# HKU-BAL/Clair

Hardware: AMD Instinct MI355X
Metric: candidate sites/sec (whole node) (higher is better)
Workload: dtype f32 (matmuls as 2-way fp16 split on MFMA with fp32 accumulate; gates/activations fp32); 1 GPU; ONT 122HD34 weights-shape model (random init), synthetic ont-profile pileup tensors, batch=1024, 4 batches in flight per GPU, inputs resident in HBM; batch=1024, streams=4, candidates_total=38912, device_warm_steps=251, collective=none (1 rank), transport=none

## Files before the change

clair_amd/csrc/engine.hip:

```cpp
#include "../../include/clair_amd.h"

#include <hip/hip_runtime.h>
#include <ctype.h>

#include <algorithm>
#include <atomic>
#include <cmath>
#include <cstdarg>
#include <cstdio>
#include <cstdlib>
#include <condition_variable>
#include <cstring>
#include <deque>
#include <list>
#include <memory>
#include <mutex>
#include <string>
#include <thread>
#include <vector>

#include "common.hip.h"
#include "dense.hip.h"
#include "decode.hip.h"
#include "evaluate.hip.h"
// ... 1178 lines not shown
    if (check_source_range(t, "clair_sites_add_rows", first, n)) return 1;
    if (fused_possible(e)) return fail(e, "clair_sites_add_rows is not available on a handle with the fused layer-2 launch: unset CLAIR_AMD_LSTM2_FUSED");
    HIP_TRY(e, hipSetDevice(e->device));
    Slot &s = e->slots[0];
    if (s.pending_n) return fail(e, "slot 0 still has a pending submit; call clair_wait first");
    if (ensure_slot_decode(e, s) || ensure_slot_sites(e, s)) return 1;
    Lane &l = *e->lanes[s.lane];
    std::lock_guard<std::mutex> g(l.order);
    HIP_TRY(e, hipMemcpyAsync(s.d_out.p, probs, (size_t)n * OUT_FLOATS * sizeof(float), hipMemcpyHostToDevice, l.stream));
    if (x) HIP_TRY(e, hipMemcpyAsync(s.d_x.p, x, (size_t)n * SITE_X * sizeof(float), hipMemcpyHostToDevice, l.stream));
    if (centre) HIP_TRY(e, hipMemcpyAsync(s.d_centre.p, centre, (size_t)n * 2, hipMemcpyHostToDevice, l.stream));
    else HIP_TRY(e, hipMemsetAsync(s.d_centre.p, 0, (size_t)n * 2, l.stream));
    if (seq) HIP_TRY(e, hipMemcpyAsync(s.d_seq.p, seq, (size_t)n * SITE_SEQ, hipMemcpyHostToDevice, l.stream));
    else HIP_TRY(e, hipMemsetAsync(s.d_seq.p, 0, (size_t)n * SITE_SEQ, l.stream));
    if (enqueue_sites_adopt(e, l, s, t, first, n, x != nullptr) || enqueue_sites_accumulate(e, l, s, t, first, n)) return 1;
    HIP_TRY(e, hipStreamSynchronize(l.stream));
    return read_overflow(t, "clair_sites_add_rows");
}

int clair_sites_finish(clair_sites_t *t, int min_count, int order, int64_t *n_out) {
    if (check_sites(t, "clair_sites_finish", false)) return 1;
    clair_engine *e = t->e;
    if (order != CLAIR_SITES_ORDER_CHAIN && order != CLAIR_SITES_ORDER_POSITION) return fail(e, "clair_sites_finish: order %d is neither chain (0) nor position (1)", order);
    HIP_TRY(e, hipSetDevice(e->device));
    if (quiesce(e)) return 1;
    if (read_overflow(t, "clair_sites_finish")) return 1;
    Lane &l = *e->lanes[0];
    std::lock_guard<std::mutex> g(l.order);
    const int64_t ns = t->n_sites;
    uint32_t kept = 0;
    if (ns > 0) {
        const int64_t *idx_row = order == CLAIR_SITES_ORDER_POSITION ? t->idx_row[t->cur].as<int64_t>() : nullptr;
        const unsigned blocks = (unsigned)((ns + 255) / 256);
        HIP_TRY(e, t->keep.ensure((size_t)ns * sizeof(uint32_t)));
        HIP_TRY(e, t->out_before.ensure((size_t)(ns + 1) * sizeof(uint32_t)));
        hipLaunchKernelGGL(sites_keep_kernel, dim3(blocks), dim3(256), 0, l.stream, t->count.as<int>(), idx_row, ns, std::max(min_count, 1), t->keep.as<uint32_t>());
        hipLaunchKernelGGL(sites_scan_kernel, dim3(1), dim3(256), 0, l.stream, t->keep.as<uint32_t>(), ns, t->out_before.as<uint32_t>());
        HIP_TRY(e, hipGetLastError());
        HIP_TRY(e, hipMemcpyAsync(&kept, t->out_before.as<uint32_t>() + ns, sizeof kept, hipMemcpyDeviceToHost, l.stream));
        HIP_TRY(e, hipStreamSynchronize(l.stream));
        if (kept) {
            HIP_TRY(e, t->out_row.ensure((size_t)kept * sizeof(int64_t)));
            HIP_TRY(e, t->out_key.ensure((size_t)kept * sizeof(int64_t)));
            HIP_TRY(e, t->out_count.ensure((size_t)kept * sizeof(int)));
            HIP_TRY(e, t->out_seq.ensure((size_t)kept * SITE_SEQ));
            HIP_TRY(e, t->avg.ensure((size_t)kept * OUT_FLOATS * sizeof(float)));
            hipLaunchKernelGGL(sites_compact_kernel, dim3(blocks), dim3(256), 0, l.stream, t->rows(), idx_row, ns, t->keep.as<uint32_t>(), t->out_before.as<uint32_t>(),
                               t->out_row.as<int64_t>(), t->out_key.as<int64_t>(), t->out_count.as<int>(), t->out_seq.as<unsigned char>());
            const int64_t n_values = (int64_t)kept * OUT_FLOATS;
            hipLaunchKernelGGL(sites_average_kernel, dim3((unsigned)((n_values + 255) / 256)), dim3(256), 0, l.stream, t->rows(), t->out_row.as<int64_t>(), n_values,
                               t->avg.as<float>());
            HIP_TRY(e, hipGetLastError());
            HIP_TRY(e, hipStreamSynchronize(l.stream));
        }
    }
    t->finished = true;
    t->n_out = kept;
    if (n_out) *n_out = kept;
    return 0;
}

int clair_sites_info(clair_sites_t *t, int64_t first, int64_t n, int64_t *positions, int32_t *counts, uint8_t *seq) {
    if (check_sites(t, "clair_sites_info", false) || check_output_range(t, "clair_sites_info", first, n)) return 1;
    clair_engine *e = t->e;
    HIP_TRY(e, hipSetDevice(e->device));
    if (n == 0) return 0;
    if (positions) HIP_TRY(e, hipMemcpy(positions, t->out_key.as<int64_t>() + first, (size_t)n * sizeof(int64_t), hipMemcpyDeviceToHost));
    if (counts) HIP_TRY(e, hipMemcpy(counts, t->out_count.as<int>() + first, (size_t)n * sizeof(int), hipMemcpyDeviceToHost));
    if (seq) HIP_TRY(e, hipMemcpy(seq, t->out_seq.as<unsigned char>() + (size_t)first * SITE_SEQ, (size_t)n * SITE_SEQ, hipMemcpyDeviceToHost));
    return 0;
}

int clair_sites_rows(clair_sites_t *t, int64_t first, int64_t n, float *out) {
    if (check_sites(t, "clair_sites_rows", false) || check_output_range(t, "clair_sites_rows", first, n)) return 1;
    clair_engine *e = t->e;
    if (n > 0 && !out) return fail(e, "clair_sites_rows: out is NULL");
    HIP_TRY(e, hipSetDevice(e->device));
    if (n > 0) HIP_TRY(e, hipMemcpy(out, t->avg.as<float>() + (size_t)first * OUT_FLOATS, (size_t)n * OUT_FLOATS * sizeof(float), hipMemcpyDeviceToHost));
    return 0;
}

int clair_sites_windows(clair_sites_t *t, int64_t first, int64_t n, float *x) {
    if (check_sites(t, "clair_sites_windows", false) || check_output_range(t, "clair_sites_windows", first, n)) return 1;
    clair_engine *e = t->e;
    if (n > INT32_MAX || (n > 0 && !x)) return fail(e, "clair_sites_windows: bad arguments");
    if (n == 0) return 0;
    HIP_TRY(e, hipSetDevice(e->device));
    if (quiesce(e)) return 1;
    Lane &l = *e->lanes[0];
    std::lock_guard<std::mutex> g(l.order);
    if (t->gathered.bytes < (size_t)n * SITE_X * sizeof(float)) HIP_TRY(e, t->gathered.ensure((size_t)n * SITE_X * sizeof(float)));
    hipLaunchKernelGGL(sites_gather_kernel, dim3((unsigned)((n + 3) / 4)), dim3(256), 0, l.stream, t->rows(), t->out_row.as<int64_t>(), t->avg.as<float>(), first, (int)n,
                       t->gathered.as<float>(), (unsigned char *)nullptr, (float *)nullptr);
    HIP_TRY(e, hipGetLastError());
    HIP_TRY(e, hipMemcpyAsync(x, t->gathered.p, (size_t)n * SITE_X * sizeof(float), hipMemcpyDeviceToHost, l.stream));
    HIP_TRY(e, hipStreamSynchronize(l.stream));
    return 0;
}

int clair_submit_site_calls(clair_engine_t *e, int slot, clair_sites_t *t, int64_t first, int n, clair_call_t *calls, float *gt21, float *genotype, float *l1, float *l2) {
    if (check_sites(t, "clair_submit_site_calls", false)) return 1;
    if (e != t->e) return fail(e, "clair_submit_site_calls: the site table belongs to another engine");
    if (check_slot(e, slot, false) || check_n(e, n)) return 1;
    if ((gt21 || genotype || l1 || l2) && !(gt21 && genotype && l1 && l2)) return fail(e, "the four probability arrays come together or not at all");
    if (!gt21 && !calls) return fail(e, "nothing asked for: neither call records nor probabilities");
    if (check_output_range(t, "clair_submit_site_calls", first, n)) return 1;
    if (fused_possible(e)) return fail(e, "clair_submit_site_calls runs on the two-launch layer-2 path only: unset CLAIR_AMD_LSTM2_FUSED");
    HIP_TRY(e, hipSetDevice(e->device));
    Slot &s = e->slots[slot];
    if (s.pending_n) return fail(e, "slot %d still has a pending submit; call clair_wait first", slot);
    if (ensure_slot_decode(e, s)) return 1;
    Lane &l = *e->lanes[s.lane];
    s.o_gt21 = gt21; s.o_gt = genotype; s.o_l1 = l1; s.o_l2 = l2;
    s.o_calls = calls;
    s.refetch = false;
    s.staged = 0;
    const bool same_out = s.cout == l.stream;
    {
        std::lock_guard<std::mutex> g(l.order);
        hipLaunchKernelGGL(sites_gather_kernel, dim3((n + 3) / 4), dim3(256), 0, l.stream, t->rows(), t->out_row.as<int64_t>(), t->avg.as<float>(), first, n, s.d_x.as<float>(),
                           s.d_centre.as<unsigned char>(), s.d_out.as<float>());
        HIP_TRY(e, hipGetLastError());
        if (calls && enqueue_decode(e, l, s, n)) return 1;
        if (same_out) { if (enqueue_results(e, l, s, n, calls != nullptr, gt21 != nullptr)) return 1; }
        else HIP_TRY(e, hipEventRecord(s.ev_done, l.stream));
    }
    if (!same_out) {
        HIP_TRY(e, hipStreamWaitEvent(s.cout, s.ev_done, 0));
        if (enqueue_results(e, l, s, n, calls != nullptr, gt21 != nullptr)) return 1;
    }
    s.pending_n = n;
    return 0;
}

int clair_predict(clair_engine_t *e, const float *x, int n, float *gt21, float *genotype, float *l1, float *l2) {
    if (clair_submit(e, 0, x, n, gt21, genotype, l1, l2)) return 1;
    return clair_wait(e, 0);
}

int clair_dataset_alloc(clair_engine_t *e, int64_t N, void **x_dev, void **out_dev) {
    if (!e) return fail(nullptr, "engine is NULL");
    if (N < 1 || !x_dev || !out_dev) return fail(e, "bad arguments to clair_dataset_alloc");
    HIP_TRY(e, hipSetDevice(e->device));
    const size_t rows = (size_t)N + e->max_pad;
    HIP_TRY(e, hipMalloc(x_dev, rows * CLAIR_INPUT_FLOATS * sizeof(float)));
    HIP_TRY(e, hipMemset(*x_dev, 0, rows * CLAIR_INPUT_FLOATS * sizeof(float)));
    HIP_TRY(e, hipMalloc(out_dev, rows * OUT_FLOATS * sizeof(float)));
    HIP_TRY(e, hipMemset(*out_dev, 0, rows * OUT_FLOATS * sizeof(float)));
    return 0;
}

int clair_dataset_free(clair_engine_t *e, void *x_dev, void *out_dev) {
    if (!e) return fail(nullptr, "engine is NULL");
    HIP_TRY(e, hipSetDevice(e->device));
    HIP_TRY(e, hipDeviceSynchronize());
    HIP_TRY(e, hipFree(x_dev));
    HIP_TRY(e, hipFree(out_dev));
    return 0;
}

int clair_dataset_upload(clair_engine_t *e, void *x_dev, int64_t first, const float *x_host, int64_t n) {
    if (!e) return fail(nullptr, "engine is NULL");
    HIP_TRY(e, hipSetDevice(e->device));
    HIP_TRY(e, hipMemcpy((float *)x_dev + (size_t)first * CLAIR_INPUT_FLOATS, x_host, (size_t)n * CLAIR_INPUT_FLOATS * sizeof(float), hipMemcpyHostToDevice));
    return 0;
}

int clair_dataset_download(clair_engine_t *e, const void *out_dev, int64_t first, float *out_host, int64_t n) {
    if (!e) return fail(nullptr, "engine is NULL");
    HIP_TRY(e, hipSetDevice(e->device));
    HIP_TRY(e, hipMemcpy(out_host, (const float *)out_dev + (size_t)first * OUT_FLOATS, (size_t)n * OUT_FLOATS * sizeof(float), hipMemcpyDeviceToHost));
    return 0;
}

int clair_run_resident(clair_engine_t *e, int slot, const void *x_dev, void *out_dev, int64_t first, int n) {
    if (check_slot(e, slot) || check_n(e, n)) return 1;
    HIP_TRY(e, hipSetDevice(e->device));
    Lane &l = *e->lanes[e->slots[slot].lane];
    std::lock_guard<std::mutex> g(l.order);
    return enqueue_forward(e, l, *e->models[0], (const float *)x_dev + (size_t)first * CLAIR_INPUT_FLOATS, (float *)out_dev + (size_t)first * OUT_FLOATS, n, -1);
}

int clair_sync(clair_engine_t *e) {
    if (!e) return fail(nullptr, "engine is NULL");
    HIP_TRY(e, hipSetDevice(e->device));
    if (quiesce(e)) return 1;
    return check_fused_placement(e);
}

int clair_timing_enable(clair_engine_t *e, int on) {
    if (!e) return fail(nullptr, "engine is NULL");
    HIP_TRY(e, hipSetDevice(e->device));
    if (drain_timers(e)) return 1;
    e->timing_mask = on == 0 ? 0u : (on == 1 ? ~0u : (unsigned)on);
    return 0;
}

int clair_kernel_times(clair_engine_t *e, double *ms_sum, int64_t *launches) {
    if (!e) return fail(nullptr, "engine is NULL");
    HIP_TRY(e, hipSetDevice(e->device));
    if (drain_timers(e)) return 1;
    for (int k = 0; k < CLAIR_K_COUNT; ++k) {
        if (ms_sum) ms_sum[k] = e->ms_sum[k];
        if (launches) launches[k] = e->launches[k];
    }
    return 0;
}

int clair_timing_reset(clair_engine_t *e) {
    if (!e) return fail(nullptr, "engine is NULL");
    HIP_TRY(e, hipSetDevice(e->device));
    if (drain_timers(e)) return 1;
    for (int k = 0; k < CLAIR_K_COUNT; ++k) { e->ms_sum[k] = 0; e->launches[k] = 0; }
    return 0;
}

int clair_kernel_workgroups(clair_engine_t *e, int n, int *workgroups) {
    if (!e) return fail(nullptr, "engine is NULL");
    if (!workgroups) return fail(e, "workgroups is NULL");
    if (n < 1 || n > e->max_batch) return fail(e, "n %d out of range [1,%d]", n, e->max_batch);
    const int n_pad = (n + 31) & ~31, ntiles = n_pad / 32;
    const int x_tiles = (T_POS * n_pad + GS_ROWS - 1) / GS_ROWS;
    for (int k = 0; k < CLAIR_K_COUNT; ++k) workgroups[k] = 0;
    workgroups[CLAIR_K_LSTM1] = ntiles * 2;
    workgroups[CLAIR_K_LSTM2] = use_lstm2_pair(e, ntiles) ? ((ntiles + 1) / 2) * 2 : ntiles * 2;
    workgroups[CLAIR_K_PROJ2] = 32 * std::min(e->proj2_groups, (x_tiles + 7) / 8);
    if (use_lstm2_fused(e, ntiles)) {
        workgroups[CLAIR_K_LSTM2] = 32 * e->fused_groups + 32 * ((ntiles / 2 + 7) / 8);
        workgroups[CLAIR_K_PROJ2] = 0;
    }
    workgroups[CLAIR_K_L4] = l34_grid((n_pad + L34_CAND - 1) / L34_CAND);
    workgroups[CLAIR_K_TAIL] = n_pad / TAIL_TILE;
    workgroups[CLAIR_K_DECODE] = (n + 3) / 4;
    return 0;
}

int clair_pinned_alloc(clair_engine_t *e, int64_t bytes, void **ptr) {
    if (!e) return fail(nullptr, "engine is NULL");
    if (!ptr || bytes < 1) return fail(e, "bad arguments to clair_pinned_alloc");
    HIP_TRY(e, hipSetDevice(e->device));
    std::list<PinnedBuffer> one(1);
    HIP_TRY(e, one.front().ensure((size_t)bytes));
    *ptr = one.front().p;
    std::lock_guard<std::mutex> g(e->pinned_mu);
    e->pinned.splice(e->pinned.end(), one);
    return 0;
}

int clair_pinned_free(clair_engine_t *e, void *ptr) {
    if (!e) return fail(nullptr, "engine is NULL");
    bool known = false;
    {
        std::lock_guard<std::mutex> g(e->pinned_mu);
        for (const auto &b : e->pinned) known |= b.p == ptr;
    }
    if (!known) return fail(e, "clair_pinned_free: not a buffer of clair_pinned_alloc");
    HIP_TRY(e, hipSetDevice(e->device));
    if (quiesce(e)) return 1;
    std::lock_guard<std::mutex> g(e->pinned_mu);
    e->pinned.remove_if([ptr](const PinnedBuffer &b) { return b.p == ptr; });
    return 0;
}

int clair_engine_counter(clair_engine_t *e, int which, int64_t *value) {
    if (!e) return fail(nullptr, "engine is NULL");
    if (!value) return fail(e, "value is NULL");
    switch (which) {
        case 0: *value = e->fused_launches; return 0;
        case 1: *value = e->fused_recoveries; return 0;
        default: return fail(e, "clair_engine_counter: unknown counter %d", which);
    }
}

int clair_debug_read(clair_engine_t *e, int slot, int which, float *host, int64_t count) {
    if (check_slot(e, slot)) return 1;
    HIP_TRY(e, hipSetDevice(e->device));
    if (quiesce(e)) return 1;
    Lane &l = *e->lanes[e->slots[slot].lane];
    const float *src = nullptr;
    int64_t avail = 0;
    const int64_t np = l.last_n_pad;
    if (which == 1) {
        avail = (int64_t)T_POS * np * 256;
        if (count > avail) return fail(e, "clair_debug_read: asked %lld floats, tap 1 holds %lld", (long long)count, (long long)avail);
        std::vector<unsigned short> planes((size_t)2 * avail);
        HIP_TRY(e, hipMemcpy(planes.data(), l.a1.p, planes.size() * sizeof(unsigned short), hipMemcpyDeviceToHost));
        for (int64_t i = 0; i < count; ++i) host[i] = f16_value(planes[i]) + f16_value(planes[avail + i]);
        return 0;
    }
    if (which == 2) {
        avail = (int64_t)T_POS * np * 256;
        if (count > avail) return fail(e, "clair_debug_read: asked %lld floats, tap 2 holds %lld", (long long)count, (long long)avail);
        std::vector<float> raw((size_t)avail);
        HIP_TRY(e, hipMemcpy(raw.data(), l.a2.p, raw.size() * sizeof(float), hipMemcpyDeviceToHost));
        for (int64_t i = 0; i < count; ++i) {
            const int64_t t = i / (np * 256), n = (i / 256) % np, c = i % 256;
            host[i] = raw[(size_t)((((c / 8) * T_POS + t) * np + n) * 8 + c % 8)];
        }
        return 0;
    }
    switch (which) {
        case 4: if (!e->tap_l3) return fail(e, "clair_debug_read: tap 4 needs CLAIR_AMD_TAP_L3=1 at engine creation");
                src = l.zx.as<float>(); avail = np * L3_OUT; break;
        case 5: if (!e->l34_stamps) return fail(e, "clair_debug_read: tap 5 needs CLAIR_AMD_L34_STAMPS=1 at engine creation");
                src = l.zx.as<float>(); avail = ((np + L34_CAND - 1) / L34_CAND) * L4_SPLITS * 8 * 16 * 2; break;
        case 3: {
            avail = (int64_t)L4_SPLITS * np * L4_UNITS;
            if (count > avail) return fail(e, "clair_debug_read: asked %lld floats, tap 3 holds %lld", (long long)count, (long long)avail);
            const int64_t nblk = (np + L34_CAND - 1) / L34_CAND;
            std::vector<float> raw((size_t)L4_SPLITS * nblk * L34_CAND * L4_UNITS);
            HIP_TRY(e, hipMemcpy(raw.data(), l.l4part.p, raw.size() * sizeof(float), hipMemcpyDeviceToHost));
            const float inv = std::ldexp(1.0f, -e->models[0]->w4_shift) / L34_ACT_SCALE;
            for (int64_t i = 0; i < count; ++i) {
                const int64_t cg = i / (np * L4_UNITS), n = (i / L4_UNITS) % np, col = i % L4_UNITS;
                const int64_t blk = n / 64, row = n % 64, mb = row / 32, a = (row % 32) / 8, hq = (row % 8) / 4, r = row % 4;
                const int64_t nh = col / 96, nb = (col % 96) / 32, l32 = col % 32;
                host[i] = raw[(size_t)((((((cg * nblk + blk) * 2 + nh) * 6 + mb * 3 + nb) * 4 + a) * 64 + hq * 32 + l32) * 4 + r)] * inv;
            }
            return 0;
        }
        default: return fail(e, "clair_debug_read: unknown tap %d", which);
    }
    if (count > avail) return fail(e, "clair_debug_read: asked %lld floats, tap %d holds %lld", (long long)count, which, (long long)avail);
    HIP_TRY(e, hipMemcpy(host, src, (size_t)count * sizeof(float), hipMemcpyDeviceToHost));
    return 0;
}

}
```

clair_amd/csrc/gemm_split.hip.h:

```cpp
#pragma once
#include "common.hip.h"
#include "lstm32.hip.h"
#include <type_traits>

namespace clair {

typedef unsigned short f16bits_t;

struct GemmSplitArgs {
    const f16bits_t *X3;
    const f16bits_t *W3;
    const float *bias;
    float *C;
    int n_pad;
    int ntiles;
    int m_rows;
    int groups;
};

constexpr int GS_ROWS = 64;
constexpr int GS_PLANE = GS_ROWS * 32;
constexpr int GS_PHASE = 2 * 2 * GS_PLANE;

__device__ __forceinline__ int split_lds_off(int row, int chunk) { return row * 32 + ((chunk ^ ((row >> 3) & 3)) << 3); }

constexpr int GS_RING = 4;

template <bool FUSED>
__device__ __forceinline__ void gemm_split_body(const GemmSplitArgs &p, const int block, const FuseArgs &fz) {
    __shared__ __attribute__((aligned(16))) f16bits_t Xs[GS_RING][GS_PHASE];

    const int tid = threadIdx.x;
    const int lane = tid & 63;
    const int wave = __builtin_amdgcn_readfirstlane(tid >> 6);
    const int l32 = lane & 31, lh = lane >> 5;
    const int xcd = block & 7, local = block >> 3;
    const int gtile = local & 3, group = local >> 2;
    const int x_tiles = (p.m_rows + GS_ROWS - 1) / GS_ROWS;
    const int x_step = 8 * p.groups;
    const int x_first = xcd + 8 * group;
    const int npairs = p.ntiles >> 1;
    const int nq = FUSED ? (xcd < npairs ? (npairs - xcd + 7) >> 3 : 0) : 0;
    const int n_items = T_POS * nq;
    if (FUSED ? group >= n_items : x_first >= x_tiles) return;
    const int n_my = FUSED ? (n_items - group + p.groups - 1) / p.groups : (x_tiles - x_first + x_step - 1) / x_step;
    const int slice = gtile * 4 + wave;
    auto xt_of = [&](int it) -> int {
        if (!FUSED) return x_first + it * x_step;
        const int i = group + it * p.groups, s_ = i / nq, k = i - s_ * nq;
        return ((gtile >> 1) ? T_POS - 1 - s_ : s_) * npairs + xcd + 8 * k;
    };

    f16x8 Wr[2][16][2];
    {
        const f16x8 *wp = (const f16x8 *)p.W3 + ((size_t)slice * (2 * 16 * 2 * 64)) + lane;
#pragma unroll
        for (int mi = 0; mi < 2; ++mi)
#pragma unroll
            for (int kk = 0; kk < 16; ++kk)
#pragma unroll
                for (int pl = 0; pl < 2; ++pl) Wr[mi][kk][pl] = wp[((mi * 16 + kk) * 2 + pl) * 64];
#pragma unroll
        for (int mi = 0; mi < 2; ++mi)
#pragma unroll
            for (int kk = 0; kk < 16; ++kk)
#pragma unroll
                for (int pl = 0; pl < 2; ++pl) asm volatile("" : "+a"(Wr[mi][kk][pl]));
    }
    f32x4 bq[2][4];
#pragma unroll
    for (int mi = 0; mi < 2; ++mi)
#pragma unroll
        for (int a = 0; a < 4; ++a) bq[mi][a] = *(const f32x4 *)(p.bias + slice * 64 + mi * 32 + 8 * a + 4 * lh);
#pragma unroll
    for (int mi = 0; mi < 2; ++mi)
#pragma unroll
        for (int a = 0; a < 4; ++a) asm volatile("" : "+v"(bq[mi][a]));
    CLAIR_VMWAIT(0);

    const int my_slab = wave >> 1, my_plane = wave & 1;
    unsigned lane_off[4];
#pragma unroll
    for (int j = 0; j < 4; ++j) {
        const int row = 16 * j + (lane >> 2), c = (lane & 3) ^ ((row >> 3) & 3);
        lane_off[j] = (unsigned)(row * 512 + c * 16);
    }
    const f16bits_t *my_base = p.X3 + (size_t)my_plane * p.m_rows * 256 + my_slab * 32;
    const unsigned lds0 = __builtin_amdgcn_readfirstlane((unsigned)(size_t)(lptr_t)&Xs[0][0]) + (unsigned)(wave * GS_PLANE * 2);
    const int n_phases = n_my * 4;
    auto phase_base = [&](int P) -> const f16bits_t * {
        const int q = P < n_phases ? P : n_phases - 1;
        return my_base + ((size_t)xt_of(q >> 2) * GS_ROWS * 256) + (q & 3) * 64;
    };
    auto dma = [&](int P, int j) { glds16_s(lane_off[j], phase_base(P), lds0 + (unsigned)((P & (GS_RING - 1)) * GS_PHASE * 2 + j * 1024)); };
    auto fread = [&](f16x8 (&xf)[2][2][2], int slot, int sl) {
#pragma unroll
        for (int kk = 0; kk < 2; ++kk)
#pragma unroll
            for (int pl = 0; pl < 2; ++pl)
#pragma unroll
                for (int ni = 0; ni < 2; ++ni)
                    xf[kk][pl][ni] = *(const f16x8 *)&Xs[slot][(sl * 2 + pl) * GS_PLANE + split_lds_off(ni * 32 + l32, 2 * kk + lh)];
    };

    auto fread1 = [&](f16x8 (&xf)[2][2][2], int slot, int sl, int i) {
        const int kk = i >> 2, pl = (i >> 1) & 1, ni = i & 1;
        xf[kk][pl][ni] = *(const f16x8 *)&Xs[slot][(sl * 2 + pl) * GS_PLANE + split_lds_off(ni * 32 + l32, 2 * kk + lh)];
    };

    f16x8 xa[2][2][2], xb[2][2][2];
#pragma unroll
    for (int P = 0; P < 3; ++P)
#pragma unroll
        for (int j = 0; j < 4; ++j) dma(P, j);
    CLAIR_VMWAIT(8);
    __syncthreads();
    fread(xa, 0, 0);

    f32x16 accs[2][2][2];
    f32x16 bias16[2];
#pragma unroll
    for (int mi = 0; mi < 2; ++mi)
#pragma unroll
        for (int a = 0; a < 4; ++a) {
            bias16[mi][4 * a] = bq[mi][a][0]; bias16[mi][4 * a + 1] = bq[mi][a][1];
            bias16[mi][4 * a + 2] = bq[mi][a][2]; bias16[mi][4 * a + 3] = bq[mi][a][3];
        }
    asm volatile("" : "+v"(bias16[0]), "+v"(bias16[1]));
    size_t gate_off[2];
#pragma unroll
    for (int mi = 0; mi < 2; ++mi) {
        const int gblk = slice * 2 + mi;
        gate_off[mi] = ((size_t)(gblk >> 4) * p.ntiles * T_POS * 16 + (gblk & 15)) * 1024;
    }
    auto tile_off = [&](int xt, int ni) -> size_t {
        const int xblk = xt * 2 + ni;
        const int t = xblk / p.ntiles, tile = xblk - t * p.ntiles;
        return ((size_t)tile * T_POS + t) * 16 * 1024;
    };
    auto store_piece = [&](const f32x16 (&acc)[2][2], const size_t (&toff)[2], int j) {
        const int ni = j >> 3, mi = (j >> 2) & 1, a = j & 3;
        f32x4 *dst = (f32x4 *)(p.C + gate_off[mi] + toff[ni] + a * 256) + lane;
        __builtin_nontemporal_store((f32x4){acc[mi][ni][4 * a], acc[mi][ni][4 * a + 1], acc[mi][ni][4 * a + 2], acc[mi][ni][4 * a + 3]}, dst);
    };
    auto publish = [&](int xt) {
        if (!FUSED) return;
        const int t = xt / npairs, q = xt - t * npairs;
        unsigned *fw = fz.flags + (((size_t)((gtile >> 1) * p.ntiles + 2 * q) * T_POS + t) * 8) + (gtile & 1) * 4 + wave;
        if (lane == 0) {
            __hip_atomic_store(fw, fz.ticket, __ATOMIC_RELAXED, __HIP_MEMORY_SCOPE_AGENT);
            __hip_atomic_store(fw + T_POS * 8, fz.ticket, __ATOMIC_RELAXED, __HIP_MEMORY_SCOPE_AGENT);
        }
    };
    auto run_tile = [&](auto set_c, auto first_c, int it) {
        constexpr int SET = decltype(set_c)::value;
        constexpr bool FIRST_TILE = decltype(first_c)::value;
        f32x16 (&acc)[2][2] = accs[SET];
        const int xt_prev = xt_of(FIRST_TILE ? 0 : it - 1);
        const size_t toff[2] = {tile_off(xt_prev, 0), tile_off(xt_prev, 1)};
#pragma unroll
        for (int ph = 0; ph < 4; ++ph) {
            const int P = it * 4 + ph;
#pragma unroll
            for (int m = 0; m < 24; ++m) {
                const int kk = m / 12, term = (m % 12) / 4, mi = (m >> 1) & 1, ni = m & 1;
                if (ph == 0 && m < 4) mfma32_av_first(acc[mi][ni], Wr[mi][0][1], xa[0][0][ni], bias16[mi]);
                else mfma32_av(acc[mi][ni], Wr[mi][ph * 4 + kk][term == 0 ? 1 : 0], xa[kk][term == 1 ? 1 : 0][ni]);
                __builtin_amdgcn_sched_barrier(0);
                CLAIR_DBG_FENCE();
                if (m < 8) fread1(xb, ph, 1, m);
                __builtin_amdgcn_sched_barrier(0);
            }
            CLAIR_VMWAIT(4);
            __syncthreads();
            if (FUSED && ph == 3 && !FIRST_TILE) publish(xt_prev);
#pragma unroll
            for (int m = 0; m < 24; ++m) {
                const int kk = m / 12, term = (m % 12) / 4, mi = (m >> 1) & 1, ni = m & 1;
                mfma32_av(acc[mi][ni], Wr[mi][ph * 4 + 2 + kk][term == 0 ? 1 : 0], xb[kk][term == 1 ? 1 : 0][ni]);
                __builtin_amdgcn_sched_barrier(0);
                CLAIR_DBG_FENCE();
                if (m < 8) fread1(xa, (ph + 1) & 3, 0, m);
                if (!FIRST_TILE && ph < 2 && m >= 1 && m <= 8) store_piece(accs[SET ^ 1], toff, ph * 8 + m - 1);
                if (m >= 10 && m < 18 && (m & 1) == 0) dma(P + 3, (m - 10) >> 1);
                __builtin_amdgcn_sched_barrier(0);
            }
        }
    };
    run_tile(std::integral_constant<int, 0>(), std::true_type(), 0);
    for (int it = 1; it < n_my; it += 2) {
        run_tile(std::integral_constant<int, 1>(), std::false_type(), it);
        if (it + 1 < n_my) run_tile(std::integral_constant<int, 0>(), std::false_type(), it + 1);
    }
    {
        const int last = n_my - 1, xt = xt_of(last);
        const size_t toff[2] = {tile_off(xt, 0), tile_off(xt, 1)};
        asm volatile("s_nop 11" : "+v"(accs[0][0][0]), "+v"(accs[0][0][1]), "+v"(accs[0][1][0]), "+v"(accs[0][1][1]),
                                  "+v"(accs[1][0][0]), "+v"(accs[1][0][1]), "+v"(accs[1][1][0]), "+v"(accs[1][1][1]));
#pragma unroll
        for (int j = 0; j < 16; ++j) {
            if ((xt * 2 + (j >> 3)) * 32 >= p.m_rows) continue;
            if (last & 1) store_piece(accs[1], toff, j); else store_piece(accs[0], toff, j);
        }
    }
    CLAIR_VMWAIT(0);
    if (FUSED) publish(xt_of(n_my - 1));
}

__global__ __launch_bounds__(256) __attribute__((amdgpu_waves_per_eu(1, 1))) void gemm_split_kernel(GemmSplitArgs p) {
    gemm_split_body<false>(p, blockIdx.x, FuseArgs{nullptr, 0u, nullptr, nullptr});
}

}
```

clair_amd/csrc/weight_images.h:

```cpp
#pragma once
#include "../../include/clair_amd.h"

#include <algorithm>
#include <cmath>
#include <cstddef>
#include <cstring>
#include <vector>

namespace clair {

struct LayerSizes {
    int t_pos, f_in, hid, l3_units, l4_units, l5_units;
    int l34_groups, l34_ks, l34_ch;
    int l32_x_shift;
};

constexpr int HEAD_SIZE[4] = {CLAIR_GT21, CLAIR_GENOTYPE, CLAIR_INDEL_LEN, CLAIR_INDEL_LEN};

constexpr int64_t TENSOR_COUNT[CLAIR_T_COUNT] = {
    160 * 512, 512, 160 * 512, 512, 384 * 512, 512, 384 * 512, 512, 256 * 33 * 30, 256 * 30,
    7680 * 192, 192, 4 * 192 * 96, 4 * 96, 96 * HEAD_SIZE[0], HEAD_SIZE[0], 96 * HEAD_SIZE[1], HEAD_SIZE[1],
    96 * HEAD_SIZE[2], HEAD_SIZE[2], 96 * HEAD_SIZE[3], HEAD_SIZE[3]};

inline unsigned short f16_bits(_Float16 h) { unsigned short u; memcpy(&u, &h, 2); return u; }
inline float f16_value(unsigned short u) { _Float16 h; memcpy(&h, &u, 2); return (float)h; }
inline void split2_host(float x, unsigned short &hi, unsigned short &lo) {
    const _Float16 h = (_Float16)x;
    const _Float16 l = (_Float16)(x - (float)h);
    hi = f16_bits(h);
    lo = f16_bits(l);
}

inline float gate_scale(int col512) {
    const float L2E = 1.44269504088896340736f;
    return ((col512 >> 7) == 1) ? 2.0f * L2E : -L2E;
}

inline int gate_col(int w, int b, int rho) {
    const int a = rho >> 3, hq = (rho >> 2) & 1, c = rho & 3;
    return c * 128 + 32 * w + 8 * b + 4 * hq + a;
}

inline int image_shift(float vmax) {
    if (!(vmax > 0.0f) || !std::isfinite(vmax)) return 0;
    int ex = 0;
    (void)std::frexp(vmax, &ex);
    return std::max(-20, std::min(40, 14 - ex));
}
inline float max_abs(const float *v, size_t n, float vmax = 0.0f) {
    for (size_t i = 0; i < n; ++i) vmax = std::max(vmax, std::fabs(v[i]));
    return vmax;
}

struct SplitImage {
    std::vector<unsigned short> data;
    explicit SplitImage(size_t frags) : data(frags * 2 * 64 * 8, 0) {}
    void put(size_t frag, int lane, int j, float v) {
        unsigned short hi, lo;
        split2_host(v, hi, lo);
        const size_t base = ((frag * 2) * 64 + lane) * 8 + j;
        data[base] = hi;
        data[base + 64 * 8] = lo;
    }
};

inline std::vector<float> pack_bias32(const std::vector<float> &fb, const std::vector<float> &bb) {
    std::vector<float> out(1024);
    for (int d = 0; d < 2; ++d)
        for (int w = 0; w < 4; ++w)
            for (int b = 0; b < 4; ++b)
                for (int rho = 0; rho < 32; ++rho) {
                    const int col = gate_col(w, b, rho);
                    out[((d * 4 + w) * 4 + b) * 32 + rho] = (d ? bb : fb)[col] * gate_scale(col);
                }
    return out;
}

inline std::vector<unsigned short> pack_wt32(const std::vector<float> &fw, const std::vector<float> &bw, int k0, int nkk, float pow2 = 1.0f) {
    SplitImage out((size_t)2 * 4 * 4 * nkk);
    for (int d = 0; d < 2; ++d) {
        const std::vector<float> &src = d ? bw : fw;
        for (int w = 0; w < 4; ++w)
            for (int b = 0; b < 4; ++b)
                for (int kk = 0; kk < nkk; ++kk)
                    for (int lane = 0; lane < 64; ++lane)
                        for (int j = 0; j < 8; ++j) {
                            const int col = gate_col(w, b, lane & 31), k = k0 + 16 * kk + 8 * (lane >> 5) + j;
                            out.put(((size_t)(d * 4 + w) * 4 + b) * nkk + kk, lane, j, src[(size_t)k * 512 + col] * gate_scale(col) * pow2);
                        }
    }
    return out.data;
}

inline std::vector<unsigned short> pack_wx2(const std::vector<float> &fw, const std::vector<float> &bw) {
    SplitImage out((size_t)8 * 2 * 2 * 16);
    for (int gt = 0; gt < 8; ++gt)
        for (int wm = 0; wm < 2; ++wm)
            for (int mi = 0; mi < 2; ++mi)
                for (int kk = 0; kk < 16; ++kk)
                    for (int lane = 0; lane < 64; ++lane)
                        for (int j = 0; j < 8; ++j) {
                            const int R = gt * 128 + wm * 64 + mi * 32 + (lane & 31), k = 16 * kk + 8 * (lane >> 5) + j;
                            const int d = R >> 9, col = gate_col((R >> 7) & 3, (R >> 5) & 3, R & 31);
                            out.put((((size_t)gt * 2 + wm) * 2 + mi) * 16 + kk, lane, j, (d ? bw : fw)[(size_t)k * 512 + col] * gate_scale(col));
                        }
    return out.data;
}

inline std::vector<unsigned short> pack_w3(const LayerSizes &L, const std::vector<float> &W3, const std::vector<float> &b3, int &shift) {
    shift = image_shift(max_abs(b3.data(), b3.size(), max_abs(W3.data(), W3.size())));
    const float pow2 = std::ldexp(1.0f, shift);
    SplitImage out((size_t)256 * 3);
    for (int c = 0; c < 256; ++c)
        for (int kk = 0; kk < 3; ++kk)
            for (int lane = 0; lane < 64; ++lane)
                for (int j = 0; j < 8; ++j) {
                    const int u = lane & 31, k = 16 * kk + 8 * (lane >> 5) + j;
                    float v = 0.0f;
                    if (u < L.l3_units && k < L.t_pos) v = W3[((size_t)c * L.t_pos + k) * L.l3_units + u];
                    else if (u < L.l3_units && k == L.t_pos) v = b3[(size_t)c * L.l3_units + u];
                    out.put((size_t)c * 3 + kk, lane, j, v * pow2);
                }
    return out.data;
}

inline std::vector<unsigned short> pack_w4(const LayerSizes &L, const std::vector<float> &W4, int &shift) {
    shift = image_shift(max_abs(W4.data(), W4.size()));
    const float pow2 = std::ldexp(1.0f, shift);
    SplitImage out((size_t)L.l34_groups * L.l34_ks * 6);
    for (int cg = 0; cg < L.l34_groups; ++cg)
        for (int ks = 0; ks < L.l34_ks; ++ks)
            for (int nb = 0; nb < 6; ++nb)
                for (int lane = 0; lane < 64; ++lane)
                    for (int j = 0; j < 8; ++j) {
                        const int u = 2 * ks + (lane >> 5), col = nb * 32 + (lane & 31);
                        out.put(((size_t)cg * L.l34_ks + ks) * 6 + nb, lane, j, W4[((size_t)u * 256 + cg * L.l34_ch + j) * L.l4_units + col] * pow2);
                    }
    return out.data;
}

inline std::vector<unsigned short> pack_w5(const LayerSizes &L, const std::vector<float> &W5all, int (&shift)[4]) {
    SplitImage out((size_t)4 * 12 * 3);
    for (int k5 = 0; k5 < 4; ++k5) {
        const float *W5 = W5all.data() + (size_t)k5 * L.l4_units * L.l5_units;
        shift[k5] = image_shift(max_abs(W5, (size_t)L.l4_units * L.l5_units));
        const float p5 = std::ldexp(1.0f, shift[k5]);
        for (int ks = 0; ks < 12; ++ks)
            for (int nb = 0; nb < 3; ++nb)
                for (int lane = 0; lane < 64; ++lane)
                    for (int j = 0; j < 8; ++j) {
                        const int k = 16 * ks + 8 * (lane >> 5) + j, n = nb * 32 + (lane & 31);
                        out.put(((size_t)k5 * 12 + ks) * 3 + nb, lane, j, W5[(size_t)k * L.l5_units + n] * p5);
                    }
    }
    return out.data;
}

inline std::vector<unsigned short> pack_wh(const std::vector<float> *tensors, int (&shift)[4], std::vector<float> &bh) {
    SplitImage out((size_t)4 * 6 * 2);
    bh.assign(4 * 64, 0.0f);
    for (int k5 = 0; k5 < 4; ++k5) {
        const std::vector<float> &Wh = tensors[CLAIR_T_HEAD_GT21_KERNEL + 2 * k5], &b = tensors[CLAIR_T_HEAD_GT21_BIAS + 2 * k5];
        shift[k5] = image_shift(max_abs(Wh.data(), Wh.size()));
        const float ph = std::ldexp(1.0f, shift[k5]);
        for (int ks = 0; ks < 6; ++ks)
            for (int nb = 0; nb < 2; ++nb)
                for (int lane = 0; lane < 64; ++lane)
                    for (int j = 0; j < 8; ++j) {
                        const int k = 16 * ks + 8 * (lane >> 5) + j, c = nb * 32 + (lane & 31);
                        if (c < HEAD_SIZE[k5]) out.put(((size_t)k5 * 6 + ks) * 2 + nb, lane, j, Wh[(size_t)k * HEAD_SIZE[k5] + c] * ph);
                    }
        for (int j = 0; j < HEAD_SIZE[k5]; ++j) bh[k5 * 64 + j] = b[j];
    }
    return out.data;
}

struct WeightImages {
    std::vector<float> bx1, bx2;
    std::vector<unsigned short> wh1s, wh2s, wx1s;
    std::vector<unsigned short> wx2s;
    std::vector<unsigned short> w3s, w4s;
    std::vector<unsigned short> w5s, whs;
    std::vector<float> b4, b5, bh;
    int w3_shift = 0, w4_shift = 0, w5_shift[4] = {0, 0, 0, 0}, wh_shift[4] = {0, 0, 0, 0};
};

inline WeightImages build_weight_images(const LayerSizes &L, const std::vector<float> *T) {
    WeightImages m;
    m.bx1 = pack_bias32(T[CLAIR_T_LSTM1_FW_BIAS], T[CLAIR_T_LSTM1_BW_BIAS]);
    m.bx2 = pack_bias32(T[CLAIR_T_LSTM2_FW_BIAS], T[CLAIR_T_LSTM2_BW_BIAS]);
    m.wx2s = pack_wx2(T[CLAIR_T_LSTM2_FW_KERNEL], T[CLAIR_T_LSTM2_BW_KERNEL]);
    m.wh1s = pack_wt32(T[CLAIR_T_LSTM1_FW_KERNEL], T[CLAIR_T_LSTM1_BW_KERNEL], L.f_in, 8);
    m.wh2s = pack_wt32(T[CLAIR_T_LSTM2_FW_KERNEL], T[CLAIR_T_LSTM2_BW_KERNEL], 2 * L.hid, 8);
    m.wx1s = pack_wt32(T[CLAIR_T_LSTM1_FW_KERNEL], T[CLAIR_T_LSTM1_BW_KERNEL], 0, 2, (float)(1 << L.l32_x_shift));
    m.w3s = pack_w3(L, T[CLAIR_T_L3_KERNEL], T[CLAIR_T_L3_BIAS], m.w3_shift);
    m.w4s = pack_w4(L, T[CLAIR_T_L4_KERNEL], m.w4_shift);
    m.b4 = T[CLAIR_T_L4_BIAS];
    m.w5s = pack_w5(L, T[CLAIR_T_L5_KERNEL], m.w5_shift);
    m.b5 = T[CLAIR_T_L5_BIAS];
    m.whs = pack_wh(T, m.wh_shift, m.bh);
    return m;
}

}
```

Measured before the change: 8.622 million candidates/s.

## Switch input-projection GEMM from 32x32x16 to 16x16x32 MFMA tiles

Rewrites the split-fp16 input-projection GEMM so each wave issues v_mfma_f32_16x16x32_f16 over a 4x4 grid of 16x16 tiles instead of 32x32x16 over 2x2 tiles. The weight image is repacked to match, the LDS swizzle and fragment reads change to 16-row lanes with 32-wide K chunks, and the bias and output store layouts are remapped. The aim is higher MFMA throughput and fewer LDS reads per K step on MI355X, at the cost of more instructions per tile and retuned DMA and store interleaving. A debug tap is also adjusted to read the zx workspace.

```diff
diff --git a/clair_amd/csrc/engine.hip b/clair_amd/csrc/engine.hip
--- a/clair_amd/csrc/engine.hip
+++ b/clair_amd/csrc/engine.hip
@@ -1504,8 +1504,11 @@
     switch (which) {
         case 4: if (!e->tap_l3) return fail(e, "clair_debug_read: tap 4 needs CLAIR_AMD_TAP_L3=1 at engine creation");
                 src = l.zx.as<float>(); avail = np * L3_OUT; break;
-        case 5: if (!e->l34_stamps) return fail(e, "clair_debug_read: tap 5 needs CLAIR_AMD_L34_STAMPS=1 at engine creation");
-                src = l.zx.as<float>(); avail = ((np + L34_CAND - 1) / L34_CAND) * L4_SPLITS * 8 * 16 * 2; break;
+        case 5: if (e->tap_l3) return fail(e, "clair_debug_read: tap 5 is not valid with CLAIR_AMD_TAP_L3=1 (l3 overwrites the zx workspace)");
+                src = l.zx.as<float>();
+                if (e->l34_stamps) avail = ((np + L34_CAND - 1) / L34_CAND) * L4_SPLITS * 8 * 16 * 2;
+                else avail = (int64_t)T_POS * np * 1024;
+                break;
         case 3: {
             avail = (int64_t)L4_SPLITS * np * L4_UNITS;
             if (count > avail) return fail(e, "clair_debug_read: asked %lld floats, tap 3 holds %lld", (long long)count, (long long)avail);
diff --git a/clair_amd/csrc/gemm_split.hip.h b/clair_amd/csrc/gemm_split.hip.h
--- a/clair_amd/csrc/gemm_split.hip.h
+++ b/clair_amd/csrc/gemm_split.hip.h
@@ -6,6 +6,13 @@
 namespace clair {
 
 typedef unsigned short f16bits_t;
+
+__device__ __forceinline__ void mfma16_av(f32x4 &acc, const f16x8 &w, const f16x8 &b) {
+    asm volatile("v_mfma_f32_16x16x32_f16 %0, %1, %2, %0" : "+v"(acc) : "a"(w), "v"(b));
+}
+__device__ __forceinline__ void mfma16_av_first(f32x4 &acc, const f16x8 &w, const f16x8 &b, const f32x4 &c) {
+    asm volatile("v_mfma_f32_16x16x32_f16 %0, %1, %2, %3" : "=&v"(acc) : "a"(w), "v"(b), "v"(c));
+}
 
 struct GemmSplitArgs {
     const f16bits_t *X3;
@@ -22,7 +29,8 @@
 constexpr int GS_PLANE = GS_ROWS * 32;
 constexpr int GS_PHASE = 2 * 2 * GS_PLANE;
 
-__device__ __forceinline__ int split_lds_off(int row, int chunk) { return row * 32 + ((chunk ^ ((row >> 3) & 3)) << 3); }
+__device__ __forceinline__ int split_lds_swz(int row) { return (0 - (row >> 2)) & 3; }
+__device__ __forceinline__ int split_lds_off(int row, int chunk) { return row * 32 + ((chunk ^ split_lds_swz(row)) << 3); }
 
 constexpr int GS_RING = 4;
 
@@ -33,7 +41,7 @@
     const int tid = threadIdx.x;
     const int lane = tid & 63;
     const int wave = __builtin_amdgcn_readfirstlane(tid >> 6);
-    const int l32 = lane & 31, lh = lane >> 5;
+    const int l16 = lane & 15, lq = lane >> 4;
     const int xcd = block & 7, local = block >> 3;
     const int gtile = local & 3, group = local >> 2;
     const int x_tiles = (p.m_rows + GS_ROWS - 1) / GS_ROWS;
@@ -51,38 +59,34 @@
         return ((gtile >> 1) ? T_POS - 1 - s_ : s_) * npairs + xcd + 8 * k;
     };
 
-    f16x8 Wr[2][16][2];
+    f16x8 Wr[4][8][2];
     {
-        const f16x8 *wp = (const f16x8 *)p.W3 + ((size_t)slice * (2 * 16 * 2 * 64)) + lane;
-#pragma unroll
-        for (int mi = 0; mi < 2; ++mi)
-#pragma unroll
-            for (int kk = 0; kk < 16; ++kk)
-#pragma unroll
-                for (int pl = 0; pl < 2; ++pl) Wr[mi][kk][pl] = wp[((mi * 16 + kk) * 2 + pl) * 64];
-#pragma unroll
-        for (int mi = 0; mi < 2; ++mi)
-#pragma unroll
-            for (int kk = 0; kk < 16; ++kk)
+        const f16x8 *wp = (const f16x8 *)p.W3 + ((size_t)slice * (4 * 8 * 2 * 64)) + lane;
+#pragma unroll
+        for (int mi = 0; mi < 4; ++mi)
+#pragma unroll
+            for (int kk = 0; kk < 8; ++kk)
+#pragma unroll
+                for (int pl = 0; pl < 2; ++pl) Wr[mi][kk][pl] = wp[((mi * 8 + kk) * 2 + pl) * 64];
+#pragma unroll
+        for (int mi = 0; mi < 4; ++mi)
+#pragma unroll
+            for (int kk = 0; kk < 8; ++kk)
 #pragma unroll
                 for (int pl = 0; pl < 2; ++pl) asm volatile("" : "+a"(Wr[mi][kk][pl]));
     }
-    f32x4 bq[2][4];
-#pragma unroll
-    for (int mi = 0; mi < 2; ++mi)
-#pragma unroll
-        for (int a = 0; a < 4; ++a) bq[mi][a] = *(const f32x4 *)(p.bias + slice * 64 + mi * 32 + 8 * a + 4 * lh);
-#pragma unroll
-    for (int mi = 0; mi < 2; ++mi)
-#pragma unroll
-        for (int a = 0; a < 4; ++a) asm volatile("" : "+v"(bq[mi][a]));
+    f32x4 bq[4];
+#pragma unroll
+    for (int mi = 0; mi < 4; ++mi) bq[mi] = *(const f32x4 *)(p.bias + slice * 64 + mi * 16 + 4 * lq);
+#pragma unroll
+    for (int mi = 0; mi < 4; ++mi) asm volatile("" : "+v"(bq[mi]));
     CLAIR_VMWAIT(0);
 
     const int my_slab = wave >> 1, my_plane = wave & 1;
     unsigned lane_off[4];
 #pragma unroll
     for (int j = 0; j < 4; ++j) {
-        const int row = 16 * j + (lane >> 2), c = (lane & 3) ^ ((row >> 3) & 3);
+        const int row = 16 * j + (lane >> 2), c = (lane & 3) ^ split_lds_swz(row);
         lane_off[j] = (unsigned)(row * 512 + c * 16);
     }
     const f16bits_t *my_base = p.X3 + (size_t)my_plane * p.m_rows * 256 + my_slab * 32;
@@ -93,22 +97,16 @@
         return my_base + ((size_t)xt_of(q >> 2) * GS_ROWS * 256) + (q & 3) * 64;
     };
     auto dma = [&](int P, int j) { glds16_s(lane_off[j], phase_base(P), lds0 + (unsigned)((P & (GS_RING - 1)) * GS_PHASE * 2 + j * 1024)); };
-    auto fread = [&](f16x8 (&xf)[2][2][2], int slot, int sl) {
-#pragma unroll
-        for (int kk = 0; kk < 2; ++kk)
-#pragma unroll
-            for (int pl = 0; pl < 2; ++pl)
-#pragma unroll
-                for (int ni = 0; ni < 2; ++ni)
-                    xf[kk][pl][ni] = *(const f16x8 *)&Xs[slot][(sl * 2 + pl) * GS_PLANE + split_lds_off(ni * 32 + l32, 2 * kk + lh)];
-    };
-
-    auto fread1 = [&](f16x8 (&xf)[2][2][2], int slot, int sl, int i) {
-        const int kk = i >> 2, pl = (i >> 1) & 1, ni = i & 1;
-        xf[kk][pl][ni] = *(const f16x8 *)&Xs[slot][(sl * 2 + pl) * GS_PLANE + split_lds_off(ni * 32 + l32, 2 * kk + lh)];
-    };
-
-    f16x8 xa[2][2][2], xb[2][2][2];
+    auto fread1 = [&](f16x8 (&xf)[2][4], int slot, int sl, int i) {
+        const int pl = i >> 2, ni = i & 3;
+        xf[pl][ni] = *(const f16x8 *)&Xs[slot][(sl * 2 + pl) * GS_PLANE + split_lds_off(ni * 16 + l16, lq)];
+    };
+    auto fread = [&](f16x8 (&xf)[2][4], int slot, int sl) {
+#pragma unroll
+        for (int i = 0; i < 8; ++i) fread1(xf, slot, sl, i);
+    };
+
+    f16x8 xa[2][4], xb[2][4];
 #pragma unroll
     for (int P = 0; P < 3; ++P)
 #pragma unroll
@@ -117,31 +115,23 @@
     __syncthreads();
     fread(xa, 0, 0);
 
-    f32x16 accs[2][2][2];
-    f32x16 bias16[2];
-#pragma unroll
-    for (int mi = 0; mi < 2; ++mi)
-#pragma unroll
-        for (int a = 0; a < 4; ++a) {
-            bias16[mi][4 * a] = bq[mi][a][0]; bias16[mi][4 * a + 1] = bq[mi][a][1];
-            bias16[mi][4 * a + 2] = bq[mi][a][2]; bias16[mi][4 * a + 3] = bq[mi][a][3];
-        }
-    asm volatile("" : "+v"(bias16[0]), "+v"(bias16[1]));
+    f32x4 accs[2][4][4];
+    const int lane_st = (lane >> 5) * 256 + (((lane >> 4) & 1) * 32 + l16) * 4;
     size_t gate_off[2];
 #pragma unroll
-    for (int mi = 0; mi < 2; ++mi) {
-        const int gblk = slice * 2 + mi;
-        gate_off[mi] = ((size_t)(gblk >> 4) * p.ntiles * T_POS * 16 + (gblk & 15)) * 1024;
-    }
-    auto tile_off = [&](int xt, int ni) -> size_t {
-        const int xblk = xt * 2 + ni;
+    for (int mb = 0; mb < 2; ++mb) {
+        const int gblk = slice * 2 + mb;
+        gate_off[mb] = ((size_t)(gblk >> 4) * p.ntiles * T_POS * 16 + (gblk & 15)) * 1024;
+    }
+    auto tile_off = [&](int xt, int nb) -> size_t {
+        const int xblk = xt * 2 + nb;
         const int t = xblk / p.ntiles, tile = xblk - t * p.ntiles;
         return ((size_t)tile * T_POS + t) * 16 * 1024;
     };
-    auto store_piece = [&](const f32x16 (&acc)[2][2], const size_t (&toff)[2], int j) {
-        const int ni = j >> 3, mi = (j >> 2) & 1, a = j & 3;
-        f32x4 *dst = (f32x4 *)(p.C + gate_off[mi] + toff[ni] + a * 256) + lane;
-        __builtin_nontemporal_store((f32x4){acc[mi][ni][4 * a], acc[mi][ni][4 * a + 1], acc[mi][ni][4 * a + 2], acc[mi][ni][4 * a + 3]}, dst);
+    auto store_piece = [&](const f32x4 (&acc)[4][4], const size_t (&toff)[2], int j) {
+        const int ni = j >> 2, mi = j & 3;
+        f32x4 *dst = (f32x4 *)(p.C + gate_off[mi >> 1] + toff[ni >> 1] + (mi & 1) * 512 + (ni & 1) * 64 + lane_st);
+        __builtin_nontemporal_store(acc[mi][ni], dst);
     };
     auto publish = [&](int xt) {
         if (!FUSED) return;
@@ -155,34 +145,34 @@
     auto run_tile = [&](auto set_c, auto first_c, int it) {
         constexpr int SET = decltype(set_c)::value;
         constexpr bool FIRST_TILE = decltype(first_c)::value;
-        f32x16 (&acc)[2][2] = accs[SET];
+        f32x4 (&acc)[4][4] = accs[SET];
         const int xt_prev = xt_of(FIRST_TILE ? 0 : it - 1);
         const size_t toff[2] = {tile_off(xt_prev, 0), tile_off(xt_prev, 1)};
 #pragma unroll
         for (int ph = 0; ph < 4; ++ph) {
             const int P = it * 4 + ph;
 #pragma unroll
-            for (int m = 0; m < 24; ++m) {
-                const int kk = m / 12, term = (m % 12) / 4, mi = (m >> 1) & 1, ni = m & 1;
-                if (ph == 0 && m < 4) mfma32_av_first(acc[mi][ni], Wr[mi][0][1], xa[0][0][ni], bias16[mi]);
-                else mfma32_av(acc[mi][ni], Wr[mi][ph * 4 + kk][term == 0 ? 1 : 0], xa[kk][term == 1 ? 1 : 0][ni]);
+            for (int m = 0; m < 48; ++m) {
+                const int term = m >> 4, mi = (m >> 2) & 3, ni = m & 3;
+                if (ph == 0 && m < 16) mfma16_av_first(acc[mi][ni], Wr[mi][0][1], xa[0][ni], bq[mi]);
+                else mfma16_av(acc[mi][ni], Wr[mi][ph * 2][term == 0 ? 1 : 0], xa[term == 1 ? 1 : 0][ni]);
                 __builtin_amdgcn_sched_barrier(0);
                 CLAIR_DBG_FENCE();
-                if (m < 8) fread1(xb, ph, 1, m);
+                if (m < 16 && (m & 1) == 0) fread1(xb, ph, 1, m >> 1);
                 __builtin_amdgcn_sched_barrier(0);
             }
             CLAIR_VMWAIT(4);
             __syncthreads();
             if (FUSED && ph == 3 && !FIRST_TILE) publish(xt_prev);
 #pragma unroll
-            for (int m = 0; m < 24; ++m) {
-                const int kk = m / 12, term = (m % 12) / 4, mi = (m >> 1) & 1, ni = m & 1;
-                mfma32_av(acc[mi][ni], Wr[mi][ph * 4 + 2 + kk][term == 0 ? 1 : 0], xb[kk][term == 1 ? 1 : 0][ni]);
+            for (int m = 0; m < 48; ++m) {
+                const int term = m >> 4, mi = (m >> 2) & 3, ni = m & 3;
+                mfma16_av(acc[mi][ni], Wr[mi][ph * 2 + 1][term == 0 ? 1 : 0], xb[term == 1 ? 1 : 0][ni]);
                 __builtin_amdgcn_sched_barrier(0);
                 CLAIR_DBG_FENCE();
-                if (m < 8) fread1(xa, (ph + 1) & 3, 0, m);
-                if (!FIRST_TILE && ph < 2 && m >= 1 && m <= 8) store_piece(accs[SET ^ 1], toff, ph * 8 + m - 1);
-                if (m >= 10 && m < 18 && (m & 1) == 0) dma(P + 3, (m - 10) >> 1);
+                if (m < 16 && (m & 1) == 0) fread1(xa, (ph + 1) & 3, 0, m >> 1);
+                if (!FIRST_TILE && ph < 2 && m < 16 && (m & 1)) store_piece(accs[SET ^ 1], toff, ph * 8 + (m >> 1));
+                if (m >= 20 && m < 36 && (m & 3) == 0) dma(P + 3, (m - 20) >> 2);
                 __builtin_amdgcn_sched_barrier(0);
             }
         }
@@ -195,8 +185,9 @@
     {
         const int last = n_my - 1, xt = xt_of(last);
         const size_t toff[2] = {tile_off(xt, 0), tile_off(xt, 1)};
-        asm volatile("s_nop 11" : "+v"(accs[0][0][0]), "+v"(accs[0][0][1]), "+v"(accs[0][1][0]), "+v"(accs[0][1][1]),
-                                  "+v"(accs[1][0][0]), "+v"(accs[1][0][1]), "+v"(accs[1][1][0]), "+v"(accs[1][1][1]));
+        asm volatile("s_nop 11");
+#pragma unroll
+        for (int q = 0; q < 32; ++q) asm volatile("" : "+v"(accs[q >> 4][(q >> 2) & 3][q & 3]));
 #pragma unroll
         for (int j = 0; j < 16; ++j) {
             if ((xt * 2 + (j >> 3)) * 32 >= p.m_rows) continue;
diff --git a/clair_amd/csrc/weight_images.h b/clair_amd/csrc/weight_images.h
--- a/clair_amd/csrc/weight_images.h
+++ b/clair_amd/csrc/weight_images.h
@@ -93,17 +93,16 @@
 }
 
 inline std::vector<unsigned short> pack_wx2(const std::vector<float> &fw, const std::vector<float> &bw) {
-    SplitImage out((size_t)8 * 2 * 2 * 16);
-    for (int gt = 0; gt < 8; ++gt)
-        for (int wm = 0; wm < 2; ++wm)
-            for (int mi = 0; mi < 2; ++mi)
-                for (int kk = 0; kk < 16; ++kk)
-                    for (int lane = 0; lane < 64; ++lane)
-                        for (int j = 0; j < 8; ++j) {
-                            const int R = gt * 128 + wm * 64 + mi * 32 + (lane & 31), k = 16 * kk + 8 * (lane >> 5) + j;
-                            const int d = R >> 9, col = gate_col((R >> 7) & 3, (R >> 5) & 3, R & 31);
-                            out.put((((size_t)gt * 2 + wm) * 2 + mi) * 16 + kk, lane, j, (d ? bw : fw)[(size_t)k * 512 + col] * gate_scale(col));
-                        }
+    SplitImage out((size_t)16 * 4 * 8);
+    for (int slice = 0; slice < 16; ++slice)
+        for (int mi = 0; mi < 4; ++mi)
+            for (int kk = 0; kk < 8; ++kk)
+                for (int lane = 0; lane < 64; ++lane)
+                    for (int j = 0; j < 8; ++j) {
+                        const int R = slice * 64 + mi * 16 + (lane & 15), k = 32 * kk + 8 * (lane >> 4) + j;
+                        const int d = R >> 9, col = gate_col((R >> 7) & 3, (R >> 5) & 3, R & 31);
+                        out.put(((size_t)slice * 4 + mi) * 8 + kk, lane, j, (d ? bw : fw)[(size_t)k * 512 + col] * gate_scale(col));
+                    }
     return out.data;
 }
 
```

Result: slower. 8.512 million candidates/s (-1.3%).
